# kento/TEZip

Hardware: AMD Instinct MI355X
Metric: frames/sec (predict+delta-encode), 512x512 seq (higher is better)
Workload: dtype f32; 1 GPU; 512x512x3 synthetic turbulence stack, 80 frames per GPU (ONE 80-frame sequence), SWP 20-frame windows, warm_up 0, lossy rel 1e-3, entropy remap on; PredNet (3,48,96,192) glorot seed 123

## Files before the change

### tezip_amd/csrc/tz_conv_kernels.hip.h

```cpp
#pragma once
#include <type_traits>

#include "tz_internal.h"
#include "tz_math.hip.h"

typedef float f32x4 __attribute__((ext_vector_type(4)));

enum { EPI_RAW = 0, EPI_RELU = 1, EPI_LSTM = 2, EPI_LSTM_PACKED = 3, EPI_POOL_ERR = 4, EPI_LSTM3 = 5, EPI_RAW3 = 6 };

struct ConvSrc {
    const float* p;
    long long nstride;
    int C;
    int pstride;
    int up;
    int cpt;
};

struct ConvArgs {
    ConvSrc src[2];
    int nsrc;
    int H, W, tiles_x, tiles_y, ncb;
    const float* Wp;
    const float* Wimg;
    const float* Wblk;
    const float* Wlat;
    const float* Wwino;
    int ipw;
    int wino_stride;
    int wino_first;
    const float* zero;
    int ncols;
    const float* bias;
    const float* init;
    long long init_nstride;
    int slot0;
    const float* initf;
    const float* auxf;
    int Cout;
    const float* aux;
    float* out0;
    long long out0_nstride;
    float* out1;
    long long out1_nstride;
    const int* out_idx;
    int clip1;
    int R;
    float* e0_out;
// ... 964 lines not shown
                    if (t > mx) mx = t;
                }
                const float d1 = h - mx, d2 = mx - h;
                float* o = a.out0 + (long long)n * a.out0_nstride;
                o[pp * 2 * C + col] = tz_relu(d1);
                o[pp * 2 * C + C + col] = tz_relu(d2);
            }
        }
    }
}

template <int EPI, bool UPS, int MTL>
__global__ __launch_bounds__(256) void k_convlat(const ConvArgs a) {
    convlat_body<EPI, UPS, MTL>(a, blockIdx.x);
}

template <int EA, int EB>
__global__ __launch_bounds__(256) void k_convlat_pair(const ConvArgs a, const ConvArgs b, int na) {
    if ((int)blockIdx.x < na) convlat_body<EA, false, 1>(a, blockIdx.x);
    else convlat_body<EB, false, 1>(b, blockIdx.x - na);
}

static constexpr int E8_PIECES = 11;

__device__ __forceinline__ void wait_vm_n(int n) {
    switch (n) {
        case 0: asm volatile("s_waitcnt vmcnt(0)" ::: "memory"); break;
        case 1: asm volatile("s_waitcnt vmcnt(1)" ::: "memory"); break;
        case 2: asm volatile("s_waitcnt vmcnt(2)" ::: "memory"); break;
        case 3: asm volatile("s_waitcnt vmcnt(3)" ::: "memory"); break;
        case 4: asm volatile("s_waitcnt vmcnt(4)" ::: "memory"); break;
        case 5: asm volatile("s_waitcnt vmcnt(5)" ::: "memory"); break;
        case 6: asm volatile("s_waitcnt vmcnt(6)" ::: "memory"); break;
        case 7: asm volatile("s_waitcnt vmcnt(7)" ::: "memory"); break;
        case 8: asm volatile("s_waitcnt vmcnt(8)" ::: "memory"); break;
        default: asm volatile("s_waitcnt vmcnt(9)" ::: "memory"); break;
    }
}

template <int NT>
struct C16b {
    static constexpr int NTI = NT == 1 ? 1 : 4;
    static constexpr int W8 = (18 * 64 * NTI * 4 + 1023) / 1024;
    static constexpr int WU = 16 * NTI;
    static constexpr int bufp(bool ups) {
        return !ups ? E8_PIECES + W8 : (E8_PIECES + W8 > U16_PIECES + WU ? E8_PIECES + W8 : U16_PIECES + WU);
    }
};

template <int NT, int EPI, bool UPS>
__global__ __launch_bounds__(NTHR, 6) void k_conv16b(const ConvArgs a) {
    constexpr int MAP = EPI == EPI_POOL_ERR ? MAP_POOL : (UPS ? MAP_PARITY : MAP_LINEAR);
    constexpr int NTI = C16b<NT>::NTI, W8 = C16b<NT>::W8, WU = C16b<NT>::WU, BUFP = C16b<NT>::bufp(UPS);
    constexpr int NBUF = UPS ? 2 : 1;
    static_assert((U16_PIECES + WU + 7) / 8 <= 9 && (E8_PIECES + W8 + 7) / 8 <= 9, "wait_vm_n covers at most 9 DMAs per wave in flight");
    constexpr int SCRATCH = EPI == EPI_LSTM_PACKED ? 8 * 32 * 17 : 0;
    __shared__ __attribute__((aligned(16))) float smem[NBUF * BUFP * 256 > SCRATCH ? NBUF * BUFP * 256 : SCRATCH];

    const int tid = threadIdx.x, lane = tid & 63, wv = __builtin_amdgcn_readfirstlane(tid >> 6);
    int bid = xcd_remap(blockIdx.x, gridDim.x);
    const int cb = bid % a.ncb;
    bid /= a.ncb;
    const int ntiles = a.tiles_x * a.tiles_y;
    const int tile = bid % ntiles, n = bid / ntiles;
    const int ty0 = (tile / a.tiles_x) * 16, tx0 = (tile % a.tiles_x) * 16;
    const int nblk = 1 + (UPS ? a.src[1].cpt : 0);
    const int g = lane >> 4;

    auto issue_block = [&](int b, int buf) -> int {
        float* dst = smem + buf * BUFP * 256;
        int ln = lane;
        asm volatile("" : "+v"(ln));
        const int P = b == 0 ? E8_PIECES : U16_PIECES, T = P + (b == 0 ? W8 : WU);
        const float* wsrc = b == 0 ? a.Wblk + (long long)cb * W8 * 256
                                   : a.Wblk + ((long long)a.ncb * W8 + ((long long)(b - 1) * a.ncb + cb) * WU) * 256;
        int cnt = 0;
        for (int piece = wv; piece < T; piece += 8, ++cnt) {
            if (piece >= P) {
                glds16(wsrc + (piece - P) * 256 + ln * 4, dst + piece * 256);
            } else if (b == 0) {
                const ConvSrc& s = a.src[0];
                const int i = piece * 64 + ln, q = i / NP16, slot = i - q * NP16;
                const int y = slot / PW, xs = slot - y * PW;
                const int x = MAP == MAP_PARITY ? (xs < PW / 2 ? 2 * xs : 2 * (xs - PW / 2) + 1) : xs;
                const int yy = ty0 - 1 + y, xx = tx0 - 1 + x;
                const bool ok = q < 2 && slot < PPIX && yy >= 0 && yy < a.H && xx >= 0 && xx < a.W;
                glds16(ok ? s.p + (long long)n * s.nstride + ((long long)yy * a.W + xx) * s.pstride + 4 * q : a.zero, dst + piece * 256);
            } else {
                const ConvSrc& s = a.src[1];
                const int i = piece * 64 + ln, q = i / NPU16, slot = i - q * NPU16;
                const int Y = slot / LW, X = slot - Y * LW;
                const int ly = (ty0 >> 1) - 1 + Y, lx = (tx0 >> 1) - 1 + X;
                const bool ok = slot < LPIX && ly >= 0 && ly < (a.H >> 1) && lx >= 0 && lx < (a.W >> 1);
                glds16(ok ? s.p + (long long)n * s.nstride + ((long long)ly * (a.W >> 1) + lx) * s.pstride + (b - 1) * 16 + 4 * q : a.zero,
                       dst + piece * 256);
            }
        }
        return cnt;
    };

    issue_block(0, 0);

    f32x4 acc[MT][NT];
    {
        const int col0 = cb * (NT * 16) + (lane & 15);
// ... 29 lines not shown
    const int wcls = MAP == MAP_PARITY ? (wv >> 1) : 0;
    int inflight = 0;
    if (nblk > 1) inflight = issue_block(1, 1);

    auto mfma_step = [&](const float (&fa)[MT], const float* wp) {
        float fb[4];
        if (NTI == 1) {
            fb[0] = wp[0];
        } else {
            const f32x4 t = *(const f32x4*)wp;
            fb[0] = t[0]; fb[1] = t[1]; fb[2] = t[2]; fb[3] = t[3];
        }
#pragma unroll
        for (int mt = 0; mt < MT; ++mt)
#pragma unroll
            for (int nt = 0; nt < NT; ++nt) acc[mt][nt] = __builtin_amdgcn_mfma_f32_16x16x4f32(fa[mt], fb[nt], acc[mt][nt], 0, 0, 0);
    };

    __builtin_amdgcn_s_setprio(1);
    wait_vm_n(inflight);
    wg_barrier();
    {
        const float* pa = smem;
        const float* wb = smem + E8_PIECES * 256 + lane * NTI;
#pragma unroll
        for (int tap = 0; tap < 9; ++tap) {
            const int dy = tap / 3, dx = tap % 3;
            const int xo = MAP == MAP_PARITY ? (dx == 1 ? ((wcls & 1) ? 1 - PW / 2 : PW / 2) : (dx >> 1)) : dx;
            const int toff = 4 * (dy * PW + xo);
#pragma unroll
            for (int kk = 0; kk < 2; ++kk) {
                float fa[MT];
#pragma unroll
                for (int mt = 0; mt < MT; ++mt) fa[mt] = pa[abase[mt] + toff + kk * 4 * NP16];
                mfma_step(fa, wb + (tap * 2 + kk) * 64 * NTI);
            }
        }
    }
    if (UPS) {
#pragma unroll 1
        for (int b = 1; b < nblk; ++b) {
            if (b + 1 < nblk) {
                wg_barrier();
                inflight = issue_block(b + 1, (b + 1) & 1);
            } else {
                inflight = 0;
            }
            wait_vm_n(inflight);
            wg_barrier();
            const float* pa = smem + (b & 1) * BUFP * 256;
            const float* wb = pa + U16_PIECES * 256 + lane * NTI;
#pragma unroll
            for (int tap = 0; tap < 4; ++tap) {
                const int toff = 4 * ((tap >> 1) * LW + (tap & 1));
#pragma unroll
                for (int kk = 0; kk < 4; ++kk) {
                    float fa[MT];
#pragma unroll
// ... 36 lines not shown
    }
    const int y = ty0 + py, xq = tx0 + px;
    if (y < a.H && xq < a.W) {
        const long long pix = (long long)y * a.W + xq;
        float* o = a.out0 + (long long)(a.out_idx ? a.out_idx[n] : n) * a.out0_nstride + pix * COUT;
        float v[COUT];
#pragma unroll
        for (int co = 0; co < COUT; ++co) {
            v[co] = tz_relu(acc[co]);
            if (a.clip1 && v[co] > 1.0f) v[co] = 1.0f;
            o[co] = v[co];
        }
        if (COUT == 3 && a.e0_out) {
            const int slot = a.e0_slot[n];
            if (slot >= 0) {
                float d1[3], d2[3];
#pragma unroll
                for (int c = 0; c < 3; ++c) {
                    const float h = a.e0_ahat[pix * 3 + c];
                    d1[c] = h - v[c];
                    d2[c] = v[c] - h;
                }
                float* e = a.e0_out + (long long)slot * a.e0_nstride + pix * 8;
                *(float4*)e = make_float4(tz_relu(d1[0]), tz_relu(d1[1]), tz_relu(d1[2]), tz_relu(d2[0]));
                *(float4*)(e + 4) = make_float4(tz_relu(d2[1]), tz_relu(d2[2]), 0.0f, 0.0f);
            }
        }
    }
}

template <int MAP>
__global__ __launch_bounds__(256) void k_to_fragments(const float* __restrict__ src, int H, int W, int tiles_x, int tiles_y,
                                                      int ncols, int ncb, int NT, float* __restrict__ dst) {
    const long long total = (long long)tiles_x * tiles_y * ncb * 8 * MT * NT * 256;
    for (long long i = (long long)blockIdx.x * blockDim.x + threadIdx.x; i < total; i += (long long)gridDim.x * blockDim.x) {
        const int r = (int)(i & 3), lane = (int)((i >> 2) & 63);
        long long q = i >> 8;
        const int nt = (int)(q % NT); q /= NT;
        const int mt = (int)(q % MT); q /= MT;
        const int wv = (int)(q & 7); q >>= 3;
        const int cb = (int)(q % ncb);
        const int tile = (int)(q / ncb);
        int py, px;
        row_to_patch<MAP>(wv * 32 + mt * 16 + (lane >> 4) * 4 + r, py, px);
        const int y = (tile / tiles_x) * 16 + py, x = (tile % tiles_x) * 16 + px;
        dst[i] = (y < H && x < W) ? src[((long long)y * W + x) * ncols + cb * NT * 16 + nt * 16 + (lane & 15)] : 0.0f;
    }
}
// ... 41 lines not shown
                                              int Wp, int C, int Cs, float* __restrict__ e0, int keys_only) {
    int n = blockIdx.y;
    long long npx = (long long)Hp * Wp;
    const bool key = is_key[n] != 0;
    if (keys_only && !key) return;
    const long long fi = in_idx[n];
    for (long long p = (long long)blockIdx.x * blockDim.x + threadIdx.x; p < npx; p += (long long)gridDim.x * blockDim.x) {
        int y = (int)(p / Wp), x = (int)(p - (long long)y * Wp);
        float* o = e0 + ((long long)n * npx + p) * Cs;
        if (C == 3 && Cs == 8) {
            float av[3];
#pragma unroll
            for (int c = 0; c < 3; ++c) {
                if (key) av[c] = (y < H && x < W) ? (float)frames_u8[(fi * H * W + (long long)y * W + x) * 3 + c] / 255.0f : 0.0f;
                else av[c] = in_stack[(fi * npx + p) * 3 + c];
            }
            float d1[3], d2[3];
#pragma unroll
            for (int c = 0; c < 3; ++c) {
                const float h = ahat0[p * 3 + c];
                d1[c] = h - av[c];
                d2[c] = av[c] - h;
            }
            *(float4*)o = make_float4(tz_relu(d1[0]), tz_relu(d1[1]), tz_relu(d1[2]), tz_relu(d2[0]));
            *(float4*)(o + 4) = make_float4(tz_relu(d2[1]), tz_relu(d2[2]), 0.0f, 0.0f);
            continue;
        }
        for (int c = 0; c < C; ++c) {
            float av;
            if (key) {
                av = 0.0f;
                if (y < H && x < W) av = (float)frames_u8[(fi * H * W + (long long)y * W + x) * C + c] / 255.0f;
            } else {
                av = in_stack[(fi * npx + p) * C + c];
            }
            float h = ahat0[p * C + c];
            float d1 = h - av, d2 = av - h;
            o[c] = tz_relu(d1);
            o[C + c] = tz_relu(d2);
        }
        for (int c = 2 * C; c < Cs; ++c) o[c] = 0.0f;
    }
}
```

### tezip_amd/csrc/tz_prednet.hip

```cpp
#include <algorithm>
#include <atomic>
#include <cmath>

#include "tz_conv_kernels.hip.h"
#include "tz_wino_kernels.hip.h"

struct Seg {
    int row_off, C;
    int up;
};
struct PackedConv {
    float* d_W = nullptr;
    float* d_Wimg = nullptr;
    float* d_Wblk = nullptr;
    float* d_Wlat = nullptr;
    float* d_Wwino = nullptr;
    const float* d_zero = nullptr;
    float* d_bias = nullptr;
    int nslots = 0, ncols = 0, NT = 1, ncb = 1;
    int wino_finite = 0;
    bool wino_all_finite = false;
    std::vector<Seg> segs;
};

enum { UNI_G0 = 0, UNI_C0 = 1, UNI_AHAT0 = 2 };
enum { UNI_USE_WINO_INIT = 1, UNI_USE_WINO_CELL = 2, UNI_USE_TILES = 4, UNI_USE_ALL = 7 };

struct tz_model {
    int L = 0;
    int stack[TZ_MAX_LEVELS] = {0}, rstack[TZ_MAX_LEVELS] = {0};
    std::vector<std::vector<float>> w;
    int Hp = 0, Wp = 0, maxB = 0;
    int cap = 0;
    bool prepared = false;
    float *R0[TZ_MAX_LEVELS] = {0}, *C0[TZ_MAX_LEVELS] = {0}, *Ahat0[TZ_MAX_LEVELS] = {0}, *G0[TZ_MAX_LEVELS] = {0};
    float *G0f[TZ_MAX_LEVELS] = {0}, *C0f[TZ_MAX_LEVELS] = {0};
    int ring[3][TZ_MAX_LEVELS] = {{0}};
    int tring[3][TZ_MAX_LEVELS] = {{0}};
    const float* uni[3][TZ_MAX_LEVELS] = {{0}};
    int uniform_mask = 0;
    int dead[TZ_MAX_LEVELS] = {0}, dead_gate[TZ_MAX_LEVELS] = {0}, dead_a[TZ_MAX_LEVELS] = {0};
    bool deadf[TZ_MAX_LEVELS] = {false};
    float *E[TZ_MAX_LEVELS] = {0}, *R1[TZ_MAX_LEVELS] = {0};
    float* P[TZ_MAX_LEVELS] = {0};
    int Pcap[TZ_MAX_LEVELS] = {0};
    std::vector<signed char> epart_choice;
    PackedConv a_conv[TZ_MAX_LEVELS], gate_t1[TZ_MAX_LEVELS], ahat0_t1;
    PackedConv gate_nf[TZ_MAX_LEVELS];
    float* d_zero = nullptr;
    int e0s = 0;
    int* d_idx = nullptr;
    std::vector<void*> allocs;
    const float* a_k(int l) const { return w[2 * l].data(); }
    const float* a_b(int l) const { return w[2 * l + 1].data(); }
    const float* ahat_k(int l) const { return w[2 * (L - 1) + 2 * l].data(); }
    const float* ahat_b(int l) const { return w[2 * (L - 1) + 2 * l + 1].data(); }
    int gate_base(int g) const {
        static const int pos[4] = {2, 1, 0, 3};
        return 2 * (L - 1) + 2 * L + pos[g] * 2 * L;
    }
    const float* g_k(int g, int l) const { return w[gate_base(g) + 2 * l].data(); }
    const float* g_b(int g, int l) const { return w[gate_base(g) + 2 * l + 1].data(); }
    int gate_cin(int l) const { return rstack[l] + 2 * stack[l] + (l < L - 1 ? rstack[l + 1] : 0); }
};
// ... 8 lines not shown

struct ColSrc {
    const float* kernel;
    const float* bias;
    int Cin, Cout, ch;
};

static int collapse_set(int a, int d, int out[2]) {
    if (a == 0) {
        if (d == 0) { out[0] = 0; return 1; }
        out[0] = 1; out[1] = 2; return 2;
    }
    if (d == 0) { out[0] = 0; out[1] = 1; return 2; }
    out[0] = 2; return 1;
}

static int pack_conv(tz_ctx* ctx, tz_model* m, const std::vector<Seg>& segs, const std::vector<ColSrc>& cols, int NT,
                     PackedConv* pc) {
    int ncols = (int)cols.size();
    int nslots = 0;
    for (auto& s : segs) nslots += (s.up ? 16 : 9) * ((s.C + 15) / 16);
    std::vector<float> W((size_t)std::max(nslots, 1) * 16 * ncols, 0.0f), B(ncols, 0.0f);
    int slot = 0;
    auto put = [&](const Seg& s, int c0, const int* kys, int nky, const int* kxs, int nkx) {
        for (int kc = 0; kc < 16 && c0 + kc < s.C; ++kc)
            for (int col = 0; col < ncols; ++col) {
                const ColSrc& cs = cols[col];
                if (cs.ch < 0) continue;
                float v = 0.0f;
                bool first = true;
                for (int iy = 0; iy < nky; ++iy)
                    for (int ix = 0; ix < nkx; ++ix) {
                        float w = cs.kernel[((size_t)(kys[iy] * 3 + kxs[ix]) * cs.Cin + s.row_off + c0 + kc) * cs.Cout + cs.ch];
                        v = first ? w : v + w;
                        first = false;
                    }
                W[((size_t)slot * 16 + kc) * ncols + col] = v;
            }
        ++slot;
    };
    for (auto& s : segs)
        for (int c0 = 0; c0 < s.C; c0 += 16) {
            if (!s.up) {
                for (int tap = 0; tap < 9; ++tap) {
                    int ky = tap / 3, kx = tap % 3;
                    put(s, c0, &ky, 1, &kx, 1);
                }
            } else {
                for (int tp = 0; tp < 4; ++tp)
                    for (int cls = 0; cls < 4; ++cls) {
                        int kys[2], kxs[2];
                        int nky = collapse_set(cls >> 1, tp >> 1, kys), nkx = collapse_set(cls & 1, tp & 1, kxs);
                        put(s, c0, kys, nky, kxs, nkx);
                    }
            }
        }
    for (int col = 0; col < ncols; ++col)
        if (cols[col].ch >= 0) B[col] = cols[col].bias[cols[col].ch];
    pc->nslots = nslots;
    pc->ncols = ncols;
// ... 39 lines not shown
        std::vector<float> I(((size_t)ncb * W8 + (size_t)nub * ncb * WU) * 256, 0.0f);
        auto wv = [&](int sl, int k, int cb, int nt, int lane) {
            return W[((size_t)sl * 16 + k) * ncols + cb * NT * 16 + nt * 16 + (lane & 15)];
        };
        for (int cb = 0; cb < ncb; ++cb)
            for (int tap = 0; tap < 9; ++tap)
                for (int kk = 0; kk < 2; ++kk)
                    for (int lane = 0; lane < 64; ++lane)
                        for (int nt = 0; nt < std::min(NT, NTI); ++nt)
                            I[(size_t)cb * W8 * 256 + (((size_t)tap * 2 + kk) * 64 + lane) * NTI + nt] = wv(tap, 4 * kk + (lane >> 4), cb, nt, lane);
        for (int b = 0; b < nub; ++b)
            for (int cb = 0; cb < ncb; ++cb)
                for (int tap = 0; tap < 4; ++tap)
                    for (int cls = 0; cls < 4; ++cls)
                        for (int kk = 0; kk < 4; ++kk)
                            for (int lane = 0; lane < 64; ++lane)
                                for (int nt = 0; nt < std::min(NT, NTI); ++nt)
                                    I[((size_t)ncb * W8 + ((size_t)b * ncb + cb) * WU) * 256 +
                                      ((((size_t)tap * 4 + cls) * 4 + kk) * 64 + lane) * NTI + nt] =
                                        wv(9 + 16 * b + 4 * tap + cls, 4 * kk + (lane >> 4), cb, nt, lane);
        TZ_TRY(dmalloc(ctx, m, (void**)&pc->d_Wblk, I.size() * 4));
        TZ_HIP(ctx, hipMemcpy(pc->d_Wblk, I.data(), I.size() * 4, hipMemcpyHostToDevice));
        pc->d_zero = m->d_zero;
    }
    return TZ_OK;
}

static int pack_wino(tz_ctx* ctx, tz_model* m, const std::vector<Seg>& segs, const std::vector<ColSrc>& cols, int NT, PackedConv* pc) {
    if (segs.empty() || segs[0].up || segs[0].C % 16 || (NT != 3 && NT != 4) || segs.size() > 2 ||
        (segs.size() == 2 && (!segs[1].up || segs[1].C % 16)))
        return TZ_OK;
    const int ncols = (int)cols.size(), ncb = ncols / (16 * NT);
    const int S1 = segs[0].C / 4, S2 = segs.size() == 2 ? segs[1].C / 4 : 0;
    std::vector<float> I((size_t)(S1 + S2) * ncb * 16 * 256, 0.0f);
    auto at = [&](int st, int cb, int set, int lane, int nt) -> float& {
        return I[((((size_t)cb * (S1 + S2) + st) * 16 + set) * 64 + lane) * 4 + nt];
    };
    std::vector<char> finite((size_t)segs[0].C / 16, 1);
    bool ups_finite = true;
    for (int col = 0; col < ncols; ++col) {
        const ColSrc& cs = cols[col];
        if (cs.ch < 0) continue;
        const int cb = col / (16 * NT), nt = (col % (16 * NT)) / 16, j = col % 16;
        for (int c = 0; c < segs[0].C; ++c) {
            float g[3][3], w[4][3], U[4][4];
            for (int r = 0; r < 3; ++r)
                for (int q = 0; q < 3; ++q) g[r][q] = cs.kernel[((size_t)(r * 3 + q) * cs.Cin + segs[0].row_off + c) * cs.Cout + cs.ch];
// ... 224 lines not shown
}

static int launch_conv(tz_ctx* ctx, int NT, int epi, const ConvArgs& a, int nbatch, int wino_dead = 0, const float* wino3 = nullptr) {
    tz_prof_scope ps(ctx, TZP_CONV);
    bool ups = false, fullk = true;
    for (int s = 0; s < a.nsrc; ++s) {
        ups = ups || a.src[s].up;
        fullk = fullk && (a.src[s].C % 16) == 0;
        const long long hs = a.src[s].up ? a.H >> 1 : a.H, ws = a.src[s].up ? a.W >> 1 : a.W;
        fullk = fullk && hs * ws * a.src[s].pstride * 4 < (1LL << 32);
    }
    ps.sub = TZP_CONV_GEN;
    if (epi == EPI_RELU && a.nsrc == 1 && !ups && a.src[0].C == 3 && a.Cout == 3 && ctx->conv_impl) {
        ps.sub = TZP_CONV_SMALL;
        hipLaunchKernelGGL((k_conv_small<3, 3>), dim3(a.tiles_x * a.tiles_y * nbatch), dim3(256), 0, ctx->stream, a);
        TZ_HIP(ctx, hipGetLastError());
        return TZ_OK;
    }
    if (a.Wblk && a.nsrc > 0 && !a.src[0].up && a.src[0].pstride == 8 && ctx->conv_impl) {
        const int blocks = a.ncb * a.tiles_x * a.tiles_y * nbatch;
#define TZ_CASE16B(nt, e, u)                                                                                    \
    if (NT == nt && epi == e && ups == u) {                                                                     \
        ps.sub = TZP_CONV16B;                                                                                   \
        hipLaunchKernelGGL((k_conv16b<nt, e, u>), dim3(blocks), dim3(NTHR), 0, ctx->stream, a);                 \
        TZ_HIP(ctx, hipGetLastError());                                                                         \
        return TZ_OK;                                                                                           \
    }
        TZ_CASE16B(1, EPI_LSTM_PACKED, true) TZ_CASE16B(1, EPI_LSTM_PACKED, false)
        TZ_CASE16B(1, EPI_POOL_ERR, false) TZ_CASE16B(3, EPI_POOL_ERR, false) TZ_CASE16B(4, EPI_POOL_ERR, false)
#undef TZ_CASE16B
    }
    if (a.Wwino && effective_contract(ctx) == 2 && fullk && (epi == EPI_LSTM || epi == EPI_POOL_ERR || epi == EPI_RAW)) {
        ps.sub = TZP_WINO;
        return launch_wino(ctx, NT, epi, ups, a, nbatch, false, wino_dead, wino3);
    }
    {
        const LatPlan lp = lat_plan(ctx, NT, epi, ups, fullk, a, nbatch);
        if (!lp.use) goto no_lat;
        const bool wide = lp.wide;
        const int blocks = lp.blocks;
        ps.sub = TZP_CONVLAT;
#define TZ_LAT(e, u)                                                                                          \
    do {                                                                                                      \
        if (wide) hipLaunchKernelGGL((k_convlat<e, u, 2>), dim3(blocks), dim3(256), 0, ctx->stream, a);       \
        else hipLaunchKernelGGL((k_convlat<e, u, 1>), dim3(blocks), dim3(256), 0, ctx->stream, a);            \
    } while (0)
        if (epi == EPI_LSTM && ups) TZ_LAT(EPI_LSTM, true);
// ... 18 lines not shown
    }
#define TZ_CASE(nt, e, u)                                                   \
    if (NT == nt && epi == e && ups == u) {                                 \
        if (fullk) launch_conv_t<nt, e, u, true>(ctx, a, nbatch);           \
        else launch_conv_t<nt, e, u, false>(ctx, a, nbatch);                \
        TZ_HIP(ctx, hipGetLastError());                                     \
        return TZ_OK;                                                       \
    }
    TZ_CASE(1, EPI_RAW, false) TZ_CASE(4, EPI_RAW, false)
    TZ_CASE(1, EPI_RELU, false) TZ_CASE(3, EPI_RELU, false) TZ_CASE(4, EPI_RELU, false)
    TZ_CASE(4, EPI_LSTM, false) TZ_CASE(4, EPI_LSTM, true)
    TZ_CASE(1, EPI_LSTM_PACKED, false) TZ_CASE(1, EPI_LSTM_PACKED, true)
    TZ_CASE(1, EPI_POOL_ERR, false) TZ_CASE(3, EPI_POOL_ERR, false) TZ_CASE(4, EPI_POOL_ERR, false)
#undef TZ_CASE
    return tz_fail(ctx, TZ_ERR_UNSUPPORTED, "no conv kernel for NT=%d epilogue=%d upsampled=%d", NT, epi, (int)ups);
}

static void fill_srcs(ConvArgs& a, const PackedConv& pc, const float* const* ptrs, const long long* nstrides,
                      int pstride0 = 0) {
    a.nsrc = (int)pc.segs.size();
    for (int s = 0; s < a.nsrc; ++s) {
        a.src[s].p = ptrs[s];
        a.src[s].nstride = nstrides[s];
        a.src[s].C = pc.segs[s].C;
        a.src[s].pstride = s == 0 && pstride0 ? pstride0 : pc.segs[s].C;
        a.src[s].up = pc.segs[s].up;
        a.src[s].cpt = (pc.segs[s].C + 15) / 16;
    }
    a.Wp = pc.d_W;
    a.Wimg = pc.d_Wimg;
    a.Wblk = pc.d_Wblk;
    a.Wlat = pc.d_Wlat;
    a.Wwino = pc.d_Wwino;
    a.zero = pc.d_zero;
    a.bias = pc.d_bias;
    a.ncols = pc.ncols;
    a.ncb = pc.ncb;
}

static void set_geom(ConvArgs& a, int H, int W) {
    a.H = H;
    a.W = W;
    a.tiles_x = (W + 15) / 16;
    a.tiles_y = (H + 15) / 16;
}

void tz_model_free(tz_ctx* ctx) {
    tz_model* m = ctx->model;
    if (!m) return;
    for (void* p : m->allocs) (void)hipFree(p);
    delete m;
    ctx->model = nullptr;
}

// ... 83 lines not shown
            if ((m->uniform_mask & UNI_USE_TILES) && H >= 16 && W >= 16 &&
                tile_inside(h_ring[1][k][l], ref_tile_origin(H), ref_tile_origin(W), H, W))
                m->tring[k][l] = h_ring[1][k][l];
            if (log) {
                const int w1 = m->ring[k][l], wt = m->tring[k][l], w = wt >= 0 && (w1 < 0 || wt < w1) ? wt : w1;
                int uniform = 0, tiles = ((H + 15) / 16) * ((W + 15) / 16);
                for (int ty0 = 0; ty0 < H; ty0 += 16)
                    for (int tx0 = 0; tx0 < W; tx0 += 16) uniform += tile_inside(w1, ty0, tx0, H, W) || tile_inside(wt, ty0, tx0, H, W);
                fprintf(stderr, "[tezip] uniform constants, level %d %s (%dx%d): w %d, 16x16 tiles %d uniform %d non-uniform; one value: w %d, "
                        "repeating tiles: w %d\n", l, names[k], H, W, w, uniform, tiles - uniform, w1, wt);
            }
        }
    }
    return TZ_OK;
}

static int measure_dead(tz_ctx* ctx, tz_model* m) {
    const int L = m->L;
    const char* env = getenv("TEZIP_DEADSRC");
    const bool on = !env || atoi(env) != 0;
    const bool log = getenv("TEZIP_DEADSRC_LOG") && atoi(getenv("TEZIP_DEADSRC_LOG"));
    unsigned long long h_live[TZ_MAX_LEVELS] = {0};
    for (int l = 0; l < TZ_MAX_LEVELS; ++l) m->dead[l] = m->dead_gate[l] = m->dead_a[l] = 0;
    if (on) {
        unsigned long long* d_live = nullptr;
        TZ_TRY(dmalloc(ctx, m, (void**)&d_live, sizeof(h_live)));
        TZ_HIP(ctx, hipMemsetAsync(d_live, 0, sizeof(h_live), ctx->stream));
        for (int l = 1; l < L; ++l) {
            const long long npx = (long long)(m->Hp >> l) * (m->Wp >> l);
            const int nb = std::min(m->stack[l] / 16, 64);
            if (nb < 1) continue;
            hipLaunchKernelGGL(k_live_blocks, dim3((unsigned)std::min<long long>((npx * m->stack[l] + 255) / 256, 4096)), dim3(256), 0, ctx->stream,
                               (const unsigned*)m->Ahat0[l], npx, m->stack[l], nb, d_live + l);
            TZ_HIP(ctx, hipGetLastError());
        }
        TZ_HIP(ctx, hipMemcpyAsync(h_live, d_live, sizeof(h_live), hipMemcpyDeviceToHost, ctx->stream));
        TZ_HIP(ctx, hipStreamSynchronize(ctx->stream));
    }
    for (int l = 1; l < L; ++l) {
        const int src_blocks = 2 * m->stack[l] / 16;
        int d = 0;
        while (on && 16 * (d + 1) <= m->stack[l] && d < 64 && d + 1 < src_blocks && !((h_live[l] >> d) & 1)) ++d;
        m->dead[l] = d;
        const PackedConv* pcs[2] = {&m->gate_t1[l], l < L - 1 ? &m->a_conv[l] : nullptr};
        int* out[2] = {&m->dead_gate[l], &m->dead_a[l]};
        static const char* const names[2] = {"gates", "A"};
        for (int k = 0; k < 2; ++k) {
            if (!pcs[k] || !pcs[k]->d_Wwino) continue;
            *out[k] = pcs[k]->wino_finite >= d ? d : 0;
            if (log)
                fprintf(stderr, "[tezip] dead source, level %d %s: %d of %d leading positive-half blocks dead, %d skipped: %d of %d same-resolution stages%s\n",
                        l, names[k], d, m->stack[l] / 16, *out[k], 4 * *out[k], 2 * m->stack[l] / 4,
                        !on ? " (TEZIP_DEADSRC=0)" : (*out[k] < d ? " (a weight of those stages is not finite)" : ""));
        }
    }
    return TZ_OK;
}

static int measure_deadf(tz_ctx* ctx, tz_model* m) {
    const int L = m->L;
    const char* env = getenv("TEZIP_DEADF");
    const bool on = !env || atoi(env) != 0;
    const bool log = getenv("TEZIP_DEADF_LOG") && atoi(getenv("TEZIP_DEADF_LOG"));
    unsigned long long h_live[TZ_MAX_LEVELS] = {0};
    for (int l = 0; l < TZ_MAX_LEVELS; ++l) m->deadf[l] = false;
    if (!on && !log) return TZ_OK;
    {
        unsigned long long* d_live = nullptr;
        TZ_TRY(dmalloc(ctx, m, (void**)&d_live, sizeof(h_live)));
        TZ_HIP(ctx, hipMemsetAsync(d_live, 0, sizeof(h_live), ctx->stream));
        for (int l = 1; l < L; ++l) {
            const long long nwords = (long long)(m->Hp >> l) * (m->Wp >> l) * m->rstack[l];
            hipLaunchKernelGGL(k_live_blocks, dim3((unsigned)std::min<long long>((nwords + 255) / 256, 4096)), dim3(256), 0, ctx->stream,
                               (const unsigned*)m->C0[l], nwords, 1, 1, d_live + l, 0xffffffffu);
            TZ_HIP(ctx, hipGetLastError());
        }
// ... 127 lines not shown
        fill_srcs(a, pc, ptrs, ns);
        set_geom(a, hl(l), wl(l));
        a.Cout = Cout;
        a.out0 = m->Ahat0[l];
        a.clip1 = l == 0;
        TZ_TRY(launch_conv(ctx, NT, EPI_RELU, a, 1));
    }
    for (int l = 0; l < L; ++l) {
        std::vector<ColSrc> cols;
        int NT;
        TZ_TRY(gate_cols(ctx, m, l, &cols, &NT));
        PackedConv pg;
        TZ_TRY(pack_conv(ctx, m, {Seg{0, m->rstack[l], 0}}, cols, NT, &pg));
        size_t npx = (size_t)hl(l) * wl(l);
        TZ_TRY(dmalloc(ctx, m, (void**)&m->G0[l], npx * pg.ncols * 4));
        ConvArgs a;
        memset(&a, 0, sizeof(a));
        const float* ptrs[2] = {m->R0[l], nullptr};
        long long ns[2] = {0, 0};
        fill_srcs(a, pg, ptrs, ns);
        set_geom(a, hl(l), wl(l));
        a.out0 = m->G0[l];
        TZ_TRY(launch_conv(ctx, NT, EPI_RAW, a, 1));
        std::vector<Seg> segs = {Seg{m->rstack[l], 2 * m->stack[l], 0}};
        if (l < L - 1) segs.push_back(Seg{m->rstack[l] + 2 * m->stack[l], m->rstack[l + 1], 1});
        TZ_TRY(pack_conv(ctx, m, segs, cols, NT, &m->gate_t1[l]));
        if (l >= 1) TZ_TRY(pack_wino(ctx, m, segs, cols, NT, &m->gate_t1[l]));
        {
            const int tx = (wl(l) + 15) / 16, ty = (hl(l) + 15) / 16, ncb = pg.ncols / (16 * NT);
            const bool parity = l < L - 1;
            const size_t nf = (size_t)tx * ty * ncb * 8 * 2 * NT * 256;
            TZ_TRY(dmalloc(ctx, m, (void**)&m->G0f[l], nf * 4));
            if (parity) hipLaunchKernelGGL(k_to_fragments<MAP_PARITY>, dim3(1024), dim3(256), 0, ctx->stream, m->G0[l], hl(l), wl(l), tx, ty, pg.ncols, ncb, NT, m->G0f[l]);
            else hipLaunchKernelGGL(k_to_fragments<MAP_LINEAR>, dim3(1024), dim3(256), 0, ctx->stream, m->G0[l], hl(l), wl(l), tx, ty, pg.ncols, ncb, NT, m->G0f[l]);
            TZ_HIP(ctx, hipGetLastError());
            if (NT == 4) {
                const size_t nc = (size_t)tx * ty * ncb * 8 * 2 * 256;
                TZ_TRY(dmalloc(ctx, m, (void**)&m->C0f[l], nc * 4));
                if (parity) hipLaunchKernelGGL(k_to_fragments<MAP_PARITY>, dim3(1024), dim3(256), 0, ctx->stream, m->C0[l], hl(l), wl(l), tx, ty, m->rstack[l], ncb, 1, m->C0f[l]);
                else hipLaunchKernelGGL(k_to_fragments<MAP_LINEAR>, dim3(1024), dim3(256), 0, ctx->stream, m->C0[l], hl(l), wl(l), tx, ty, m->rstack[l], ncb, 1, m->C0f[l]);
                TZ_HIP(ctx, hipGetLastError());
            }
        }
    }
    for (int l = 0; l < L - 1; ++l) {
        int Cout = m->stack[l + 1], NT = plain_nt(Cout);
        TZ_TRY(pack_conv(ctx, m, {Seg{0, 2 * m->stack[l], 0}}, plain_cols(m->a_k(l), m->a_b(l), 2 * m->stack[l], Cout), NT,
                         &m->a_conv[l]));
        if (l >= 1) TZ_TRY(pack_wino(ctx, m, {Seg{0, 2 * m->stack[l], 0}}, plain_cols(m->a_k(l), m->a_b(l), 2 * m->stack[l], Cout), NT, &m->a_conv[l]));
    }
    TZ_TRY(measure_uniform(ctx, m));
    TZ_TRY(measure_dead(ctx, m));
    TZ_TRY(measure_deadf(ctx, m));
    m->prepared = true;
    return TZ_OK;
}

int tz_model_dims(tz_ctx* ctx, int* Hp, int* Wp, int* max_batch) {
    tz_model* m = ctx->model;
    if (!m || !m->prepared) return tz_fail(ctx, TZ_ERR_STATE, "model not prepared");
    *Hp = m->Hp;
    *Wp = m->Wp;
    *max_batch = m->cap;
    return TZ_OK;
}

int tz_model_c0_dev(tz_ctx* ctx, const float** c0) {
    tz_model* m = ctx->model;
    if (!m || !m->prepared) return tz_fail(ctx, TZ_ERR_STATE, "model not prepared");
    *c0 = m->Ahat0[0];
// ... 129 lines not shown
    auto npx = [&](int l) { return (long long)hl(l) * wl(l); };
    if (fused_next) *fused_next = false;
    if (!skip_err0) {
        tz_prof_scope ps(ctx, TZP_ERR0);
        int gx = (int)std::min<long long>((npx(0) + 255) / 256, 2048);
        hipLaunchKernelGGL(k_err0, dim3(gx, n), dim3(256), 0, ctx->stream, d_frames_u8, H, W, d_in_stack, d_idx,
                           d_idx + stride, m->Ahat0[0], Hp, Wp, m->stack[0], m->e0s, m->E[0] + (long long)slot0 * npx(0) * m->e0s,
                           err0_keys_only ? 1 : 0);
        TZ_HIP(ctx, hipGetLastError());
    }
    auto set_uniform = [&](const float*& u, int& ring, int& tring, int k, int l, int use) {
        const bool on = (m->uniform_mask & use) && m->ring[k][l] >= 0;
        u = on ? m->uni[k][l] : nullptr;
        ring = on ? m->ring[k][l] : -1;
        tring = (m->uniform_mask & use) ? m->tring[k][l] : -1;
    };
    auto gate_args = [&](int l, ConvArgs& a) {
        const PackedConv& pc = m->gate_t1[l];
        memset(&a, 0, sizeof(a));
        const int ec = l == 0 ? m->e0s : 2 * m->stack[l];
        long long ns[2] = {npx(l) * ec, l < L - 1 ? npx(l + 1) * m->rstack[l + 1] : 0};
        const float* ptrs[2] = {m->E[l] + slot0 * ns[0], l < L - 1 ? m->R1[l + 1] + slot0 * ns[1] : nullptr};
        fill_srcs(a, pc, ptrs, ns, ec);
        set_geom(a, hl(l), wl(l));
        a.init = m->G0[l];
        a.initf = m->G0f[l];
        a.Cout = m->rstack[l];
        a.R = m->rstack[l];
        a.aux = m->C0[l];
        a.auxf = m->C0f[l];
        a.out0_nstride = npx(l) * m->rstack[l];
        a.out0 = m->R1[l] + slot0 * a.out0_nstride;
        set_uniform(a.init_u, a.init_ring, a.init_tring, UNI_G0, l, l >= 1 ? UNI_USE_WINO_INIT : 0);
        set_uniform(a.aux_u, a.aux_ring, a.aux_tring, UNI_C0, l, l >= 1 ? UNI_USE_WINO_CELL : 0);
    };
    auto aconv_args = [&](int l, ConvArgs& a) {
        const PackedConv& pc = m->a_conv[l];
        memset(&a, 0, sizeof(a));
        const int ec = l == 0 ? m->e0s : 2 * m->stack[l];
        long long ns[2] = {npx(l) * ec, 0};
        const float* ptrs[2] = {m->E[l] + slot0 * ns[0], nullptr};
        fill_srcs(a, pc, ptrs, ns, ec);
        set_geom(a, hl(l), wl(l));
        a.Cout = m->stack[l + 1];
        a.aux = m->Ahat0[l + 1];
        a.init_tring = a.aux_tring = -1;
        a.out0_nstride = npx(l + 1) * 2 * m->stack[l + 1];
        a.out0 = m->E[l + 1] + slot0 * a.out0_nstride;
    };
    bool epart[TZ_MAX_LEVELS] = {false};
    if (use_epart) {
        double idle;
        epart_levels(ctx, m, n, epart, &idle);
    }
    auto wino3 = [&](int l) -> const float* { return m->deadf[l] ? m->gate_nf[l].d_Wwino : nullptr; };
    auto pcols = [&](int l) { return m->deadf[l] ? 3 * m->rstack[l] : m->gate_t1[l].ncols; };
    auto epart_launch = [&](int l) -> int {
        if (!ctx->ev_epart_src[l]) {
            TZ_HIP(ctx, hipEventCreateWithFlags(&ctx->ev_epart_src[l], hipEventDisableTiming));
            TZ_HIP(ctx, hipEventCreateWithFlags(&ctx->ev_epart_done[l], hipEventDisableTiming));
        }
        ConvArgs ge;
        gate_args(l, ge);
        ge.wino_stride = (ge.src[0].C + ge.src[1].C) >> 2;
        ge.wino_first = 0;
// ... 122 lines not shown
}

extern "C" int tz_predict_c0(tz_ctx* ctx, float* out) {
    if (!ctx || !out) return TZ_ERR_INVALID;
    const float* c0;
    TZ_TRY(tz_model_c0_dev(ctx, &c0));
    tz_model* m = ctx->model;
    size_t bytes = (size_t)m->Hp * m->Wp * m->stack[0] * 4;
    TZ_HIP(ctx, hipMemcpyAsync(out, c0, bytes, hipMemcpyDefault, ctx->stream));
    if (!tz_is_device_ptr(out)) TZ_HIP(ctx, hipStreamSynchronize(ctx->stream));
    return TZ_OK;
}

extern "C" int tz_predict_next(tz_ctx* ctx, const float* frames, int n, float* out) {
    if (!ctx || !frames || !out || n < 0) return TZ_ERR_INVALID;
    tz_model* m = ctx->model;
    if (!m || !m->prepared) return tz_fail(ctx, TZ_ERR_STATE, "model not prepared");
    size_t fe = (size_t)m->Hp * m->Wp * m->stack[0];
    tz_call call(ctx);
    const float* din;
    float* dout;
    TZ_TRY(call.in(frames, fe * n * 4, &din));
    TZ_TRY(call.out(out, fe * n * 4, &dout));
    for (int b0 = 0; b0 < n; b0 += m->maxB) {
        int nb = std::min(m->maxB, n - b0);
        std::vector<int> isk(nb, 0), ii(nb), oi(nb);
        for (int i = 0; i < nb; ++i) ii[i] = oi[i] = b0 + i;
        TZ_TRY(tz_model_predict_batch(ctx, nb, isk.data(), ii.data(), oi.data(), nullptr, 0, 0, din, dout));
    }
    return call.finish();
}

__global__ __launch_bounds__(256) void k_act_probe(const float* __restrict__ x, size_t n, float* __restrict__ hs,
                                                   float* __restrict__ th) {
    const size_t stride = (size_t)gridDim.x * blockDim.x;
    for (size_t i = (size_t)blockIdx.x * blockDim.x + threadIdx.x; i < n; i += stride) {
        hs[i] = tz_hard_sigmoid(x[i]);
        th[i] = tz_tanh(x[i]);
    }
}

__global__ __launch_bounds__(256) void k_recip_check(unsigned lo_bits, unsigned hi_bits, unsigned long long* __restrict__ bad) {
    const unsigned stride = gridDim.x * blockDim.x;
    unsigned long long mine = 0;
    for (unsigned long long b = (unsigned long long)lo_bits + blockIdx.x * blockDim.x + threadIdx.x; b <= hi_bits; b += stride) {
        const float d = __uint_as_float((unsigned)b);
// ... 20 lines not shown
        TZ_TRY(call.finish());
    }
    if (recip_mismatches) {
        unsigned long long* d_bad;
        TZ_TRY(call.alloc(8, &d_bad));
        TZ_HIP(ctx, hipMemsetAsync(d_bad, 0, 8, ctx->stream));
        hipLaunchKernelGGL(k_recip_check, dim3(4096), dim3(256), 0, ctx->stream, 0x40800000u, 0x4D000000u, d_bad);
        TZ_HIP(ctx, hipGetLastError());
        TZ_HIP(ctx, hipMemcpyAsync(recip_mismatches, d_bad, 8, hipMemcpyDeviceToHost, ctx->stream));
        TZ_HIP(ctx, hipStreamSynchronize(ctx->stream));
    }
    return TZ_OK;
}

extern "C" int tz_predict_tap(tz_ctx* ctx, int kind, int level, float* out) {
    if (!ctx || !out) return TZ_ERR_INVALID;
    tz_model* m = ctx->model;
    if (!m || !m->prepared) return tz_fail(ctx, TZ_ERR_STATE, "model not prepared");
    if (level < 0 || level >= m->L || kind < 0 || kind > 1) return tz_fail(ctx, TZ_ERR_INVALID, "bad tap");
    size_t npx = (size_t)(m->Hp >> level) * (m->Wp >> level);
    const float* src = kind == 0 ? m->E[level] : m->R1[level];
    const size_t ch = kind == 0 ? 2 * m->stack[level] : m->rstack[level];
    const size_t sch = kind == 0 && level == 0 ? m->e0s : ch;
    TZ_HIP(ctx, hipMemcpy2DAsync(out, ch * 4, src, sch * 4, ch * 4, npx, hipMemcpyDefault, ctx->stream));
    TZ_HIP(ctx, hipStreamSynchronize(ctx->stream));
    return TZ_OK;
}
```

Before: 3174 frames/s.

## Skip dead positive-half E0 k-step in level-0 conv16b when Ahat0 is zero

```diff
diff --git a/tezip_amd/csrc/tz_conv_kernels.hip.h b/tezip_amd/csrc/tz_conv_kernels.hip.h
--- a/tezip_amd/csrc/tz_conv_kernels.hip.h
+++ b/tezip_amd/csrc/tz_conv_kernels.hip.h
@@ -24,6 +24,7 @@
     const float* Wp;
     const float* Wimg;
     const float* Wblk;
+    const float* Wblk0;
     const float* Wlat;
     const float* Wwino;
     int ipw;
@@ -1034,6 +1035,7 @@
 }
 
 static constexpr int E8_PIECES = 11;
+static constexpr int E4_PIECES = 6;
 
 __device__ __forceinline__ void wait_vm_n(int n) {
     switch (n) {
@@ -1054,18 +1056,22 @@
 struct C16b {
     static constexpr int NTI = NT == 1 ? 1 : 4;
     static constexpr int W8 = (18 * 64 * NTI * 4 + 1023) / 1024;
+    static constexpr int W8D = (9 * 64 * NTI * 4 + 1023) / 1024;
     static constexpr int WU = 16 * NTI;
-    static constexpr int bufp(bool ups) {
-        return !ups ? E8_PIECES + W8 : (E8_PIECES + W8 > U16_PIECES + WU ? E8_PIECES + W8 : U16_PIECES + WU);
+    static constexpr int bufp(bool ups, bool dead0) {
+        const int b0 = dead0 ? E4_PIECES + W8D : E8_PIECES + W8;
+        return !ups ? b0 : (b0 > U16_PIECES + WU ? b0 : U16_PIECES + WU);
     }
 };
 
-template <int NT, int EPI, bool UPS>
+template <int NT, int EPI, bool UPS, bool DEAD0 = false>
 __global__ __launch_bounds__(NTHR, 6) void k_conv16b(const ConvArgs a) {
     constexpr int MAP = EPI == EPI_POOL_ERR ? MAP_POOL : (UPS ? MAP_PARITY : MAP_LINEAR);
-    constexpr int NTI = C16b<NT>::NTI, W8 = C16b<NT>::W8, WU = C16b<NT>::WU, BUFP = C16b<NT>::bufp(UPS);
+    constexpr int NTI = C16b<NT>::NTI, W8 = C16b<NT>::W8, WU = C16b<NT>::WU, BUFP = C16b<NT>::bufp(UPS, DEAD0);
+    constexpr int P0 = DEAD0 ? E4_PIECES : E8_PIECES, W0 = DEAD0 ? C16b<NT>::W8D : W8;
+    constexpr int KS0 = DEAD0 ? 1 : 2;
     constexpr int NBUF = UPS ? 2 : 1;
-    static_assert((U16_PIECES + WU + 7) / 8 <= 9 && (E8_PIECES + W8 + 7) / 8 <= 9, "wait_vm_n covers at most 9 DMAs per wave in flight");
+    static_assert((U16_PIECES + WU + 7) / 8 <= 9 && (P0 + W0 + 7) / 8 <= 9, "wait_vm_n covers at most 9 DMAs per wave in flight");
     constexpr int SCRATCH = EPI == EPI_LSTM_PACKED ? 8 * 32 * 17 : 0;
     __shared__ __attribute__((aligned(16))) float smem[NBUF * BUFP * 256 > SCRATCH ? NBUF * BUFP * 256 : SCRATCH];
 
@@ -1083,8 +1089,8 @@
         float* dst = smem + buf * BUFP * 256;
         int ln = lane;
         asm volatile("" : "+v"(ln));
-        const int P = b == 0 ? E8_PIECES : U16_PIECES, T = P + (b == 0 ? W8 : WU);
-        const float* wsrc = b == 0 ? a.Wblk + (long long)cb * W8 * 256
+        const int P = b == 0 ? P0 : U16_PIECES, T = P + (b == 0 ? W0 : WU);
+        const float* wsrc = b == 0 ? (DEAD0 ? a.Wblk0 : a.Wblk) + (long long)cb * W0 * 256
                                    : a.Wblk + ((long long)a.ncb * W8 + ((long long)(b - 1) * a.ncb + cb) * WU) * 256;
         int cnt = 0;
         for (int piece = wv; piece < T; piece += 8, ++cnt) {
@@ -1092,7 +1098,7 @@
                 glds16(wsrc + (piece - P) * 256 + ln * 4, dst + piece * 256);
             } else if (b == 0) {
                 const ConvSrc& s = a.src[0];
-                const int i = piece * 64 + ln, q = i / NP16, slot = i - q * NP16;
+                const int i = piece * 64 + ln, q = DEAD0 ? 1 : i / NP16, slot = DEAD0 ? i : i - q * NP16;
                 const int y = slot / PW, xs = slot - y * PW;
                 const int x = MAP == MAP_PARITY ? (xs < PW / 2 ? 2 * xs : 2 * (xs - PW / 2) + 1) : xs;
                 const int yy = ty0 - 1 + y, xx = tx0 - 1 + x;
@@ -1168,18 +1174,18 @@
     wg_barrier();
     {
         const float* pa = smem;
-        const float* wb = smem + E8_PIECES * 256 + lane * NTI;
+        const float* wb = smem + P0 * 256 + lane * NTI;
 #pragma unroll
         for (int tap = 0; tap < 9; ++tap) {
             const int dy = tap / 3, dx = tap % 3;
             const int xo = MAP == MAP_PARITY ? (dx == 1 ? ((wcls & 1) ? 1 - PW / 2 : PW / 2) : (dx >> 1)) : dx;
             const int toff = 4 * (dy * PW + xo);
 #pragma unroll
-            for (int kk = 0; kk < 2; ++kk) {
+            for (int kk = 0; kk < KS0; ++kk) {
                 float fa[MT];
 #pragma unroll
                 for (int mt = 0; mt < MT; ++mt) fa[mt] = pa[abase[mt] + toff + kk * 4 * NP16];
-                mfma_step(fa, wb + (tap * 2 + kk) * 64 * NTI);
+                mfma_step(fa, wb + (tap * KS0 + kk) * 64 * NTI);
             }
         }
     }
@@ -1262,8 +1268,8 @@
                     d2[c] = v[c] - h;
                 }
                 float* e = a.e0_out + (long long)slot * a.e0_nstride + pix * 8;
-                *(float4*)e = make_float4(tz_relu(d1[0]), tz_relu(d1[1]), tz_relu(d1[2]), tz_relu(d2[0]));
-                *(float4*)(e + 4) = make_float4(tz_relu(d2[1]), tz_relu(d2[2]), 0.0f, 0.0f);
+                *(float4*)e = make_float4(tz_relu(d1[0]), tz_relu(d1[1]), tz_relu(d1[2]), 0.0f);
+                *(float4*)(e + 4) = make_float4(tz_relu(d2[0]), tz_relu(d2[1]), tz_relu(d2[2]), 0.0f);
             }
         }
     }
@@ -1351,8 +1357,21 @@
                 d1[c] = h - av[c];
                 d2[c] = av[c] - h;
             }
-            *(float4*)o = make_float4(tz_relu(d1[0]), tz_relu(d1[1]), tz_relu(d1[2]), tz_relu(d2[0]));
-            *(float4*)(o + 4) = make_float4(tz_relu(d2[1]), tz_relu(d2[2]), 0.0f, 0.0f);
+            *(float4*)o = make_float4(tz_relu(d1[0]), tz_relu(d1[1]), tz_relu(d1[2]), 0.0f);
+            *(float4*)(o + 4) = make_float4(tz_relu(d2[0]), tz_relu(d2[1]), tz_relu(d2[2]), 0.0f);
+            continue;
+        }
+        if (Cs == 8) {
+            for (int c = 0; c < 8; ++c) o[c] = 0.0f;
+            for (int c = 0; c < C; ++c) {
+                float av = 0.0f;
+                if (!key) av = in_stack[(fi * npx + p) * C + c];
+                else if (y < H && x < W) av = (float)frames_u8[(fi * H * W + (long long)y * W + x) * C + c] / 255.0f;
+                float h = ahat0[p * C + c];
+                float d1 = h - av, d2 = av - h;
+                o[c] = tz_relu(d1);
+                o[4 + c] = tz_relu(d2);
+            }
             continue;
         }
         for (int c = 0; c < C; ++c) {
diff --git a/tezip_amd/csrc/tz_prednet.hip b/tezip_amd/csrc/tz_prednet.hip
--- a/tezip_amd/csrc/tz_prednet.hip
+++ b/tezip_amd/csrc/tz_prednet.hip
@@ -8,11 +8,16 @@
 struct Seg {
     int row_off, C;
     int up;
+    int half = 0;
+    int row(int c) const { return half && c >= half ? 4 + c - half : c; }
 };
 struct PackedConv {
     float* d_W = nullptr;
     float* d_Wimg = nullptr;
     float* d_Wblk = nullptr;
+    float* d_Wblk0 = nullptr;
+    bool pos_finite = false;
+    std::vector<float> h_W0;
     float* d_Wlat = nullptr;
     float* d_Wwino = nullptr;
     const float* d_zero = nullptr;
@@ -40,6 +45,8 @@
     const float* uni[3][TZ_MAX_LEVELS] = {{0}};
     int uniform_mask = 0;
     int dead[TZ_MAX_LEVELS] = {0}, dead_gate[TZ_MAX_LEVELS] = {0}, dead_a[TZ_MAX_LEVELS] = {0};
+    bool dead0 = false;
+    bool dead0_hold = false;
     bool deadf[TZ_MAX_LEVELS] = {false};
     float *E[TZ_MAX_LEVELS] = {0}, *R1[TZ_MAX_LEVELS] = {0};
     float* P[TZ_MAX_LEVELS] = {0};
@@ -94,6 +101,7 @@
     for (auto& s : segs) nslots += (s.up ? 16 : 9) * ((s.C + 15) / 16);
     std::vector<float> W((size_t)std::max(nslots, 1) * 16 * ncols, 0.0f), B(ncols, 0.0f);
     int slot = 0;
+    bool pos_finite = true;
     auto put = [&](const Seg& s, int c0, const int* kys, int nky, const int* kxs, int nkx) {
         for (int kc = 0; kc < 16 && c0 + kc < s.C; ++kc)
             for (int col = 0; col < ncols; ++col) {
@@ -107,7 +115,8 @@
                         v = first ? w : v + w;
                         first = false;
                     }
-                W[((size_t)slot * 16 + kc) * ncols + col] = v;
+                W[((size_t)slot * 16 + s.row(c0 + kc) - c0) * ncols + col] = v;
+                if (s.half && c0 + kc < s.half && !std::isfinite(v)) pos_finite = false;
             }
         ++slot;
     };
@@ -193,7 +202,27 @@
         TZ_TRY(dmalloc(ctx, m, (void**)&pc->d_Wblk, I.size() * 4));
         TZ_HIP(ctx, hipMemcpy(pc->d_Wblk, I.data(), I.size() * 4, hipMemcpyHostToDevice));
         pc->d_zero = m->d_zero;
-    }
+        if (segs[0].half) {
+            pc->pos_finite = pos_finite;
+            pc->h_W0.assign(W.begin(), W.begin() + (size_t)9 * 16 * ncols);
+        }
+    }
+    return TZ_OK;
+}
+
+static int pack_block0_dead(tz_ctx* ctx, tz_model* m, PackedConv* pc) {
+    if (pc->h_W0.empty() || !pc->d_Wblk) return TZ_OK;
+    const int NT = pc->NT, ncb = pc->ncb, ncols = pc->ncols, NTI = NT == 1 ? 1 : 4;
+    const int W8D = (9 * 64 * NTI * 4 + 1023) / 1024;
+    std::vector<float> I((size_t)ncb * W8D * 256, 0.0f);
+    for (int cb = 0; cb < ncb; ++cb)
+        for (int tap = 0; tap < 9; ++tap)
+            for (int lane = 0; lane < 64; ++lane)
+                for (int nt = 0; nt < std::min(NT, NTI); ++nt)
+                    I[(size_t)cb * W8D * 256 + ((size_t)tap * 64 + lane) * NTI + nt] =
+                        pc->h_W0[((size_t)tap * 16 + 4 + (lane >> 4)) * ncols + cb * NT * 16 + nt * 16 + (lane & 15)];
+    TZ_TRY(dmalloc(ctx, m, (void**)&pc->d_Wblk0, I.size() * 4));
+    TZ_HIP(ctx, hipMemcpy(pc->d_Wblk0, I.data(), I.size() * 4, hipMemcpyHostToDevice));
     return TZ_OK;
 }
 
@@ -464,7 +493,8 @@
 #define TZ_CASE16B(nt, e, u)                                                                                    \
     if (NT == nt && epi == e && ups == u) {                                                                     \
         ps.sub = TZP_CONV16B;                                                                                   \
-        hipLaunchKernelGGL((k_conv16b<nt, e, u>), dim3(blocks), dim3(NTHR), 0, ctx->stream, a);                 \
+        if (a.Wblk0) hipLaunchKernelGGL((k_conv16b<nt, e, u, true>), dim3(blocks), dim3(NTHR), 0, ctx->stream, a); \
+        else hipLaunchKernelGGL((k_conv16b<nt, e, u>), dim3(blocks), dim3(NTHR), 0, ctx->stream, a);            \
         TZ_HIP(ctx, hipGetLastError());                                                                         \
         return TZ_OK;                                                                                           \
     }
@@ -529,7 +559,7 @@
     for (int s = 0; s < a.nsrc; ++s) {
         a.src[s].p = ptrs[s];
         a.src[s].nstride = nstrides[s];
-        a.src[s].C = pc.segs[s].C;
+        a.src[s].C = pc.segs[s].half ? 8 : pc.segs[s].C;
         a.src[s].pstride = s == 0 && pstride0 ? pstride0 : pc.segs[s].C;
         a.src[s].up = pc.segs[s].up;
         a.src[s].cpt = (pc.segs[s].C + 15) / 16;
@@ -537,6 +567,7 @@
     a.Wp = pc.d_W;
     a.Wimg = pc.d_Wimg;
     a.Wblk = pc.d_Wblk;
+    a.Wblk0 = pc.d_Wblk0;
     a.Wlat = pc.d_Wlat;
     a.Wwino = pc.d_Wwino;
     a.zero = pc.d_zero;
@@ -666,11 +697,22 @@
     const bool log = getenv("TEZIP_DEADSRC_LOG") && atoi(getenv("TEZIP_DEADSRC_LOG"));
     unsigned long long h_live[TZ_MAX_LEVELS] = {0};
     for (int l = 0; l < TZ_MAX_LEVELS; ++l) m->dead[l] = m->dead_gate[l] = m->dead_a[l] = 0;
-    if (on) {
+    const char* env0 = getenv("TEZIP_DEAD0");
+    const bool on0 = !env0 || atoi(env0) != 0;
+    const bool log0 = getenv("TEZIP_DEAD0_LOG") && atoi(getenv("TEZIP_DEAD0_LOG"));
+    const bool half0 = m->e0s == 8;
+    m->dead0 = false;
+    if (on || ((on0 || log0) && half0)) {
         unsigned long long* d_live = nullptr;
         TZ_TRY(dmalloc(ctx, m, (void**)&d_live, sizeof(h_live)));
         TZ_HIP(ctx, hipMemsetAsync(d_live, 0, sizeof(h_live), ctx->stream));
-        for (int l = 1; l < L; ++l) {
+        if ((on0 || log0) && half0) {
+            const long long npx = (long long)m->Hp * m->Wp;
+            hipLaunchKernelGGL(k_live_blocks, dim3((unsigned)std::min<long long>((npx * m->stack[0] + 255) / 256, 4096)), dim3(256), 0, ctx->stream,
+                               (const unsigned*)m->Ahat0[0], npx, m->stack[0], 1, d_live);
+            TZ_HIP(ctx, hipGetLastError());
+        }
+        for (int l = 1; on && l < L; ++l) {
             const long long npx = (long long)(m->Hp >> l) * (m->Wp >> l);
             const int nb = std::min(m->stack[l] / 16, 64);
             if (nb < 1) continue;
@@ -696,6 +738,25 @@
                 fprintf(stderr, "[tezip] dead source, level %d %s: %d of %d leading positive-half blocks dead, %d skipped: %d of %d same-resolution stages%s\n",
                         l, names[k], d, m->stack[l] / 16, *out[k], 4 * *out[k], 2 * m->stack[l] / 4,
                         !on ? " (TEZIP_DEADSRC=0)" : (*out[k] < d ? " (a weight of those stages is not finite)" : ""));
+        }
+    }
+    if (half0 && (on0 || log0)) {
+        const bool zero = !(h_live[0] & 1);
+        m->dead0 = zero;
+        PackedConv* pcs[2] = {L > 1 ? &m->a_conv[0] : nullptr, &m->gate_t1[0]};
+        static const char* const names[2] = {"A", "gates"};
+        for (int k = 0; k < 2; ++k) {
+            if (!pcs[k]) continue;
+            const bool form = pcs[k]->d_Wblk && !pcs[k]->h_W0.empty() && (k == 0 || pcs[k]->NT == 1), finite = pcs[k]->pos_finite;
+            if (on0 && zero && form && finite) TZ_TRY(pack_block0_dead(ctx, m, pcs[k]));
+            if (log0)
+                fprintf(stderr, "[tezip] dead level 0, %s: positive half of E_0 +0 everywhere: %s, its k-step left out: %s%s\n", names[k],
+                        zero ? "yes" : "no", pcs[k]->d_Wblk0 ? "yes" : "no",
+                        pcs[k]->d_Wblk0 ? " (9 of 18 k-steps in block 0 of k_conv16b)"
+                        : !zero         ? ""
+                        : !on0          ? " (TEZIP_DEAD0=0)"
+                        : !form         ? " (no k_conv16b form)"
+                                        : " (a weight of those rows is not finite)");
         }
     }
     return TZ_OK;
@@ -869,7 +930,8 @@
         set_geom(a, hl(l), wl(l));
         a.out0 = m->G0[l];
         TZ_TRY(launch_conv(ctx, NT, EPI_RAW, a, 1));
-        std::vector<Seg> segs = {Seg{m->rstack[l], 2 * m->stack[l], 0}};
+        const int half = l == 0 && m->e0s == 8 ? m->stack[0] : 0;
+        std::vector<Seg> segs = {Seg{m->rstack[l], 2 * m->stack[l], 0, half}};
         if (l < L - 1) segs.push_back(Seg{m->rstack[l] + 2 * m->stack[l], m->rstack[l + 1], 1});
         TZ_TRY(pack_conv(ctx, m, segs, cols, NT, &m->gate_t1[l]));
         if (l >= 1) TZ_TRY(pack_wino(ctx, m, segs, cols, NT, &m->gate_t1[l]));
@@ -892,7 +954,8 @@
     }
     for (int l = 0; l < L - 1; ++l) {
         int Cout = m->stack[l + 1], NT = plain_nt(Cout);
-        TZ_TRY(pack_conv(ctx, m, {Seg{0, 2 * m->stack[l], 0}}, plain_cols(m->a_k(l), m->a_b(l), 2 * m->stack[l], Cout), NT,
+        const int half = l == 0 && m->e0s == 8 ? m->stack[0] : 0;
+        TZ_TRY(pack_conv(ctx, m, {Seg{0, 2 * m->stack[l], 0, half}}, plain_cols(m->a_k(l), m->a_b(l), 2 * m->stack[l], Cout), NT,
                          &m->a_conv[l]));
         if (l >= 1) TZ_TRY(pack_wino(ctx, m, {Seg{0, 2 * m->stack[l], 0}}, plain_cols(m->a_k(l), m->a_b(l), 2 * m->stack[l], Cout), NT, &m->a_conv[l]));
     }
@@ -1068,6 +1131,7 @@
         long long ns[2] = {npx(l) * ec, l < L - 1 ? npx(l + 1) * m->rstack[l + 1] : 0};
         const float* ptrs[2] = {m->E[l] + slot0 * ns[0], l < L - 1 ? m->R1[l + 1] + slot0 * ns[1] : nullptr};
         fill_srcs(a, pc, ptrs, ns, ec);
+        if (m->dead0_hold) a.Wblk0 = nullptr;
         set_geom(a, hl(l), wl(l));
         a.init = m->G0[l];
         a.initf = m->G0f[l];
@@ -1087,6 +1151,7 @@
         long long ns[2] = {npx(l) * ec, 0};
         const float* ptrs[2] = {m->E[l] + slot0 * ns[0], nullptr};
         fill_srcs(a, pc, ptrs, ns, ec);
+        if (m->dead0_hold) a.Wblk0 = nullptr;
         set_geom(a, hl(l), wl(l));
         a.Cout = m->stack[l + 1];
         a.aux = m->Ahat0[l + 1];
@@ -1255,6 +1320,22 @@
     float* dout;
     TZ_TRY(call.in(frames, fe * n * 4, &din));
     TZ_TRY(call.out(out, fe * n * 4, &dout));
+    struct Hold {
+        tz_model* m;
+        ~Hold() { m->dead0_hold = false; }
+    } hold{m};
+    if (m->dead0 && n > 0) {
+        unsigned long long* d_neg;
+        unsigned long long neg = 0;
+        TZ_TRY(call.alloc(8, &d_neg));
+        TZ_HIP(ctx, hipMemsetAsync(d_neg, 0, 8, ctx->stream));
+        hipLaunchKernelGGL(k_live_blocks, dim3((unsigned)std::min<size_t>((fe * n + 255) / 256, 4096)), dim3(256), 0, ctx->stream,
+                           (const unsigned*)din, (long long)(fe * n), 1, 1, d_neg, 0x80000000u);
+        TZ_HIP(ctx, hipGetLastError());
+        TZ_HIP(ctx, hipMemcpyAsync(&neg, d_neg, 8, hipMemcpyDeviceToHost, ctx->stream));
+        TZ_HIP(ctx, hipStreamSynchronize(ctx->stream));
+        m->dead0_hold = neg != 0;
+    }
     for (int b0 = 0; b0 < n; b0 += m->maxB) {
         int nb = std::min(m->maxB, n - b0);
         std::vector<int> isk(nb, 0), ii(nb), oi(nb);
@@ -1321,7 +1402,13 @@
     const float* src = kind == 0 ? m->E[level] : m->R1[level];
     const size_t ch = kind == 0 ? 2 * m->stack[level] : m->rstack[level];
     const size_t sch = kind == 0 && level == 0 ? m->e0s : ch;
-    TZ_HIP(ctx, hipMemcpy2DAsync(out, ch * 4, src, sch * 4, ch * 4, npx, hipMemcpyDefault, ctx->stream));
+    if (kind == 0 && level == 0 && m->e0s == 8) {
+        const size_t hb = (size_t)m->stack[0] * 4;
+        TZ_HIP(ctx, hipMemcpy2DAsync(out, ch * 4, src, sch * 4, hb, npx, hipMemcpyDefault, ctx->stream));
+        TZ_HIP(ctx, hipMemcpy2DAsync((char*)out + hb, ch * 4, src + 4, sch * 4, hb, npx, hipMemcpyDefault, ctx->stream));
+    } else {
+        TZ_HIP(ctx, hipMemcpy2DAsync(out, ch * 4, src, sch * 4, ch * 4, npx, hipMemcpyDefault, ctx->stream));
+    }
     TZ_HIP(ctx, hipStreamSynchronize(ctx->stream));
     return TZ_OK;
 }
```

Result: faster. 3254 frames/s, median of 6 (+2.5%).
